# BruceCanovas/supersurfel_fusion

Measured on AMD Instinct MI355X. Metric: frames_per_sec, higher is better.
Workload: dtype f32; 1 GPU; 640x480 synthetic RGB-D orbit (seed 1234), map seeded with 1000000 supersurfels (~993223 live, ~86081 visible), reference rgbd_benchmark parameters, extract+ICP+fuse per frame; width=640, height=480, n_model=993223, n_visible=86081, superpixels=1200, icp_iter_max=10, icp_forced=False, seed_order=seeded, exchange=none, pipeline_depth=2, extract_batch=8

## Files before the change

### supersurfel_fusion_amd/csrc/lab/host_probes.inc

```

int ssf_dbg_last_icp_record(ssf_handle* h, int64_t* out29) {
    if (!h || !out29) return SSF_ERR_INVALID_ARG;
    for (int i = 0; i < 29; i++) out29[i] = h->h_icp_local[i];
    return SSF_OK;
}
int ssf_dbg_device_icp_records(ssf_handle* h, int64_t* out64) {
    if (!h || !out64) return SSF_ERR_INVALID_ARG;
    HCK(hipStreamSynchronize(h->stream));
    HCK(hipMemcpy(out64, h->d_icp, 64 * sizeof(int64_t), hipMemcpyDeviceToHost));
    return SSF_OK;
}
void ssf_dbg_stall_before_match_us(ssf_handle* h, long long us) { if (h) h->dbg_stall_before_match_us = us; }
long long ssf_dbg_assoc_replica_frames(ssf_handle* h) { return h ? h->n_assoc_replica_frames : -1; }
int ssf_dbg_host_times(ssf_handle* h, double* out8) {
    if (!h || !out8) return SSF_ERR_INVALID_ARG;
    for (int i = 0; i < 8; i++) { out8[i] = h->host_us[i]; h->host_us[i] = 0; }
    return SSF_OK;
}
double ssf_dbg_extract_only(ssf_handle* h, const void* const* rgb, const void* const* depth, int nlist, int n) {
    if (!h || !rgb || !depth || nlist <= 0 || !h->pending.empty()) return -1.0;
    int nsub = 0;
    double t0 = 0;
    for (int i = 0; i < n; i++) {
        if (i == n / 4) { for (auto& c : h->ctx) (void)hipStreamSynchronize(c.stream); (void)hipStreamSynchronize(h->stream); t0 = now_us(); }
        while (nsub < n && !h->ctx[h->open_ctx].launched) {
            if (submit_extract(h, rgb[nsub % nlist], depth[nsub % nlist], 1, nullptr)) return -1.0;
            nsub++;
        }
        if (activate_oldest(h) || retire_active(h)) return -1.0;
        h->stamp++;
    }
    for (auto& c : h->ctx) (void)hipStreamSynchronize(c.stream);
    (void)hipStreamSynchronize(h->stream);
    return (now_us() - t0) / (double)(n - n / 4);
}
double ssf_dbg_time_icp(ssf_handle* h, int reps, int dbg) {
// ... 111 lines not shown
```

### supersurfel_fusion_amd/csrc/ssf_handle.hpp

```cpp
#pragma once
#include <algorithm>
#include <cassert>
#include <climits>
#include <cmath>
#include <cstring>
#include <deque>
#include <initializer_list>
#include <map>
#include <string>
#include <utility>
#include <vector>
#include "ssf_device.hpp"
#include "ssf_stage_layout.hpp"
#include "../../include/ssf_render.h"
#include "../../include/ssf_graph.h"
#include "../../include/ssf_graph_solve.h"
#include "../../include/ssf_keyframes.h"
#include "../../include/ssf_motion.h"
#include "../../include/ssf_odometry.h"
#include "../../include/ssf_navgrid.h"
#include "../../include/ssf_track.h"

struct ncclComm; typedef struct ncclComm* ncclComm_t;
struct Uploader;
// ... 241 lines not shown
    BinnedList bl;
    unsigned long long* stats = nullptr; int* cbox = nullptr;
    unsigned char* io = nullptr; size_t io_bytes = 0;
    RayIndex ix{};
    bool built = false; unsigned long long gen = 0; long long recentres = 0; float cell = 0, s = 0; int hash_bits = 0;
    long long rows_indexed = 0, rows_oversize = 0, entries = 0;
};
struct ssf_handle {
    ssf_config cfg;
    int S = 0, gx = 0, gy = 0;
    std::string err;
    hipStream_t stream = nullptr; bool own_stream = false; int stream_prio = 0;
    SegParams seg; Cam cam;
    std::vector<ExtractCtx> ctx; int open_ctx = 0, batch = 1;
    std::deque<std::pair<int, int>> pending;
    ActiveFrame active; ActiveFrame* cc = &active;
    uint32_t extract_ordinal = 0;
    const void* const* seq_rgb = nullptr; const void* const* seq_depth = nullptr; const uint8_t* const* seq_pixmask = nullptr; int seq_next = 0, seq_n = 0, seq_on_device = 0, stamp_bias = 0;
    long long n_waiter_matches = 0;
    int seq_k = 0;
    int seq_batches = 0;
    double us_wait_upload = 0.0;
    Uploader* up = nullptr; bool seq_upload = false;
    int in_color = SSF_COLOR_RGB8, in_depth = SSF_DEPTH_F32_METRES; double in_scale = 1.0;
    ncclComm_t comm = nullptr; int* d_all5 = nullptr;
    int deal = 0; long long deal_batches = 0;
    struct P2P {
        unsigned char* region = nullptr; size_t bytes = 0; bool fine = false;
        bool same_device = false; double timeout_s = 30.0;
        P2PView view{}; bool on = false; std::vector<void*> opened;
        unsigned long long seq_icp = 0, seq_cnt = 0, seq_assoc = 0, seq_migr = 0;
    } p2p;
    unsigned long long all_seq = 0; bool all_pending = false, all_valid = false;
    long long all_cnt[5 * SSF_MAX_RANKS];
    SurfelSoA model[2]; int mcur = 0;
    std::vector<void*> allocs;
    struct Guarded { void* base; size_t bytes, guard; };
    std::vector<Guarded> guarded;
    float* d_bf_in = nullptr; float* d_bf_out = nullptr; float* d_orient9 = nullptr; float* d_frame_orient9 = nullptr;
    long long* d_icp = nullptr;
    uint8_t* d_state = nullptr; int32_t* d_cand = nullptr; Counters* d_cnt = nullptr;
    int32_t* d_migrants = nullptr; PartitionWs fuse_ws{}; bool fuse_first = false, fuse_migrate = false, fusing = false;
    MoveTotals fuse_totals{0, 0, 0, 0}; bool move_totals_on = true;
    OovStore oov[2]; int ocur = 0; int oov_head = 0, oov_tail = 0, oov_live = 0; long long n_recentres = 0;
    uint8_t* d_state_oov = nullptr; uint32_t* d_bc_oov = nullptr;
    uint32_t* d_part = nullptr; uint32_t* d_part_ticket = nullptr; int part_words = 0, part_sup_vis = 0, part_sup_oov = 0, part_set = 0;
// ... 106 lines not shown
```

### supersurfel_fusion_amd/csrc/ssf_host.hip

```cpp
#include <atomic>
#include <chrono>
#include <cstdio>
#include <cstdlib>
#include <new>
#include <condition_variable>
#include <mutex>
#include <thread>
#include <type_traits>
#include <unistd.h>
#include "ssf_exchange.hpp"
#include "ssf_solvers.hpp"

using namespace ssf;

namespace ssf {
static thread_local KernelTimer* g_timer = nullptr;
KernelTimer* current_timer() { return g_timer; }
void set_current_timer(KernelTimer* t) { g_timer = t; }
void timer_begin(KernelTimer* t, const char* name, hipStream_t st) {
    KernelTimer::Rec r;
    if (!t->pool_free.empty()) { r = t->pool_free.back(); t->pool_free.pop_back(); }
    else { (void)hipEventCreate(&r.e0); (void)hipEventCreate(&r.e1); }
    r.name = name;
    (void)hipEventRecord(r.e0, st);
    t->open.push_back(r);
}
void timer_end(KernelTimer* t, hipStream_t st) {
    KernelTimer::Rec r = t->open.back(); t->open.pop_back();
    (void)hipEventRecord(r.e1, st);
    t->pending.push_back(r);
}
static void timer_calibrate(KernelTimer* t, hipStream_t st) {
    if (t->bracket_bias_ms >= 0.0) return;
    hipEvent_t e[2 * 16];
    for (auto& x : e) (void)hipEventCreate(&x);
    for (int i = 0; i < 16; i++) { (void)hipEventRecord(e[2 * i], st); (void)hipEventRecord(e[2 * i + 1], st); }
// ... 317 lines not shown
        NCK(api->GroupStart());
        ncclResult_t bc_rc = ncclSuccess;
        for (int b = 0; b < nb && bc_rc == ncclSuccess; b++) {
            const size_t off = (size_t)b * c.maps.slab;
            int32_t* lab = slab_shift(c.maps.label, off); float* pd = slab_shift(c.maps.plane_depth, off); float* w = slab_shift(c.d_wire, off);
            bc_rc = api->Broadcast(lab, lab, P, ncclInt32, root, c.deal_comm, st);
            if (bc_rc == ncclSuccess) bc_rc = api->Broadcast(pd, pd, P, ncclFloat32, root, c.deal_comm, st);
            if (bc_rc == ncclSuccess) bc_rc = api->Broadcast(w, w, 26 * (size_t)h->S, ncclFloat32, root, c.deal_comm, st);
        }
        const ncclResult_t end_rc = api->GroupEnd();
        if (extract_rc) return extract_rc;
        NCK(bc_rc); NCK(end_rc);
        if (!mine || h->deal == 2) launch_import_frame(st, h->seg, c.maps, nb, c.frame, c.d_wire, c.d_best, c.d_matched);
    }
    HCK(hipGetLastError());
    if (c.timed) HCK(hipEventRecord(c.ev_t1, st));
    if (multi) HCK(hipEventRecord(c.ev_done, st));
    if (multi && h->pass_team) h->team_prev = &c;
    c.launched = true; c.waited = false; c.inflight = nb; c.nb_launched = nb;
    h->open_ctx = (int)((&c - h->ctx.data() + 1) % (ptrdiff_t)h->ctx.size());
    if (h->seq_n > 0) {
        if (h->seq_launches < 32) { h->seq_launch_us[h->seq_launches] = t_launch0 - h->seq_t0_us; h->seq_launch_host_us[h->seq_launches] = now_us() - t_launch0; h->seq_launch_n[h->seq_launches++] = nb; }
        h->seq_batches++;
    }
    return SSF_OK;
}
static size_t color_bpp(const ssf_handle* h) { return (h->in_color == SSF_COLOR_RGBA8 || h->in_color == SSF_COLOR_BGRA8) ? 4 : 3; }
static size_t depth_bpp(const ssf_handle* h) { return h->in_depth == SSF_DEPTH_U16_SCALED ? 2 : 4; }
static bool device_input_aligned(ssf_handle* h, const void* rgb, const void* depth) {
    const size_t ca = color_bpp(h) == 4 ? 4 : 1, da = depth_bpp(h);
    if ((rgb && (uintptr_t)rgb % ca) || (depth && (uintptr_t)depth % da)) {
        h->err = "device frame pointer not aligned for the input format (4-byte colour: 4 bytes; depth: its element size)";
        return false;
    }
    return true;
}
static bool frame_args_ok(ssf_handle* h, const void* rgb, const void* depth, int on_device) {
    return h && rgb && depth && (!on_device || device_input_aligned(h, rgb, depth));
}
static int submit_extract(ssf_handle* h, const void* rgb, const void* depth, int on_device, const uint8_t* mask,
                          const uint8_t* pixmask = nullptr, int pixmask_on_device = 0) {
    ExtractCtx& c = h->ctx[h->open_ctx];
    if (c.launched) { h->err = "extract pipeline is full: process a submitted frame first"; return SSF_ERR_STATE; }
    if (on_device && !device_input_aligned(h, rgb, depth)) return SSF_ERR_INVALID_ARG;
    const int b = c.count;
    if (b == 0) {
        c.stamp0 = h->stamp + h->stamp_bias + (int)h->pending.size(); c.mask_bits = 0; c.pixmask_bits = 0; c.epoch0 = h->extract_ordinal;
        c.from_tables = false;
        if (h->deal && h->comm) { c.deal_batch = h->deal_batches++; c.mine = (int)(c.deal_batch % (long long)h->cfg.nranks) == h->cfg.rank; }
        else c.mine = true;
    }
    h->extract_ordinal++;
    const size_t P = (size_t)h->cfg.width * h->cfg.height, off = (size_t)b * c.maps.slab;
    c.in.rgb[b] = (const uint8_t*)rgb; c.in.depth[b] = depth;
    if (!on_device && c.mine) {
        uint8_t* drgb = slab_shift(c.d_rgb_in, off); float* ddep = slab_shift(c.d_depth_in, off);
        HCK(hipMemcpyAsync(drgb, rgb, color_bpp(h) * P, hipMemcpyHostToDevice, c.stream));
        HCK(hipMemcpyAsync(ddep, depth, depth_bpp(h) * P, hipMemcpyHostToDevice, c.stream));
        c.in.rgb[b] = drgb; c.in.depth[b] = ddep;
    }
    if (mask && c.mine) { HCK(hipMemcpyAsync(slab_shift(c.d_mask, off), mask, h->S, hipMemcpyHostToDevice, c.stream)); c.mask_bits |= 1u << b; }
    if (pixmask && c.mine) {
        HCK(hipMemcpyAsync(slab_shift(c.d_pixmask, off), pixmask, P, pixmask_on_device ? hipMemcpyDeviceToDevice : hipMemcpyHostToDevice, c.stream));
        c.pixmask_bits |= 1u << b;
    }
    c.count = b + 1;
    h->pending.push_back(std::make_pair(h->open_ctx, b));
    if (c.count == (h->seq_n > 0 ? seq_batch_size(h->seq_batches, h->batch) : h->batch)) return launch_batch(h, c);
    return SSF_OK;
}
static int submit_tables(ssf_handle* h, const int32_t* label, const float* plane_depth, const ssf_surfels* fr, int on_device) {
    if (h->ctx[h->open_ctx].count > 0 && !h->ctx[h->open_ctx].launched) {
        int rc = launch_batch(h, h->ctx[h->open_ctx]);
        if (rc) return rc;
    }
    ExtractCtx& c = h->ctx[h->open_ctx];
    if (c.launched) { h->err = "extract pipeline is full: process a submitted frame first"; return SSF_ERR_STATE; }
    hipStream_t st = c.stream;
    const bool multi = h->ctx.size() > 1;
    if (multi && c.consumed_valid) HCK(hipStreamWaitEvent(st, c.ev_consumed, 0));
    c.stamp0 = h->stamp + h->stamp_bias + (int)h->pending.size(); c.mask_bits = 0; c.pixmask_bits = 0; c.epoch0 = h->extract_ordinal;
    h->extract_ordinal++;
    c.from_tables = true;
    const size_t P = (size_t)h->cfg.width * h->cfg.height, S = (size_t)h->S;
    const hipMemcpyKind kind = on_device ? hipMemcpyDeviceToDevice : hipMemcpyHostToDevice;
    c.timed = false;
    HCK(hipMemcpyAsync(c.maps.label, label, 4 * P, kind, st));
    HCK(hipMemcpyAsync(c.maps.plane_depth, plane_depth, 4 * P, kind, st));
    float* w = c.d_wire;
    HCK(hipMemcpyAsync(w, fr->positions, 12 * S, kind, st)); w += 3 * S;
    HCK(hipMemcpyAsync(w, fr->colors, 12 * S, kind, st)); w += 3 * S;
    HCK(hipMemcpyAsync(w, fr->stamps, 8 * S, kind, st)); w += 2 * S;
    HCK(hipMemcpyAsync(w, fr->orientations, 36 * S, kind, st)); w += 9 * S;
    HCK(hipMemcpyAsync(w, fr->shapes, 24 * S, kind, st)); w += 6 * S;
    HCK(hipMemcpyAsync(w, fr->dims, 8 * S, kind, st)); w += 2 * S;
    HCK(hipMemcpyAsync(w, fr->confidences, 4 * S, kind, st));
    if (!on_device) HCK(hipStreamSynchronize(st));
    launch_import_frame(st, h->seg, c.maps, 1, c.frame, c.d_wire, c.d_best, c.d_matched);
    HCK(hipGetLastError());
    if (multi) HCK(hipEventRecord(c.ev_done, st));
    c.count = 1; c.launched = true; c.waited = false; c.inflight = 1; c.nb_launched = 1;
    h->pending.push_back(std::make_pair(h->open_ctx, 0));
    h->open_ctx = (int)((&c - h->ctx.data() + 1) % (ptrdiff_t)h->ctx.size());
    return SSF_OK;
}
static int retire_active(ssf_handle* h) {
    ExtractCtx* c = h->active.ctx;
    if (!c || !h->have_frame) return SSF_OK;
    h->have_frame = false;
    if (--c->inflight == 0) {
        if (h->ctx.size() > 1) { HCK(hipEventRecord(c->ev_consumed, h->stream)); c->consumed_valid = true; }
        c->launched = false; c->count = 0;
    }
    return SSF_OK;
}
static int activate_oldest(ssf_handle* h) {
    if (h->fusing) { h->err = "a frame is between ssf_stage_fuse_begin and ssf_stage_fuse_end"; return SSF_ERR_STATE; }
    if (h->pending.empty()) { h->err = "no submitted frame"; return SSF_ERR_STATE; }
    int rc = retire_active(h);
    if (rc) return rc;
    const std::pair<int, int> fr = h->pending.front();
    ExtractCtx& c = h->ctx[fr.first];
    if (!c.launched) { rc = launch_batch(h, c); if (rc) return rc; }
    h->pending.pop_front();
    if (h->ctx.size() > 1 && !c.waited) { HCK(hipStreamWaitEvent(h->stream, c.ev_done, 0)); c.waited = true; }
    if (c.stamp0 + fr.second != h->stamp) { h->err = "submitted frame is out of sequence (model stamp changed while frames were pending)"; return SSF_ERR_STATE; }
    const size_t off = (size_t)fr.second * c.maps.slab;
    ActiveFrame& a = h->active;
    a.maps = batch_slot(c.maps, fr.second); a.frame = batch_slot(c.frame, off);
    a.d_best = slab_shift(c.d_best, off); a.d_matched = slab_shift(c.d_matched, off);
    a.ctx = &c; a.slot = fr.second; a.pixmask = ((c.pixmask_bits >> fr.second) & 1u) != 0;
    a.has_rgba = !c.from_tables && c.mine; a.activated = true;
    h->have_frame = true;
    return SSF_OK;
}
static int seq_flush_tail(ssf_handle* h) {
    if (h->seq_next < h->seq_n) return SSF_OK;
    ExtractCtx& c = h->ctx[h->open_ctx];
    return (c.count > 0 && !c.launched) ? launch_batch(h, c) : SSF_OK;
}
static int seq_submit(ssf_handle* h) {
    const int i = h->seq_next;
    const uint8_t* pixmask = h->seq_pixmask ? h->seq_pixmask[i] : nullptr;
    if (h->seq_on_device || !h->seq_upload) {
        int rc = submit_extract(h, h->seq_rgb[i], h->seq_depth[i], h->seq_on_device, nullptr, pixmask, h->seq_on_device);
        if (!rc) { h->seq_next++; rc = seq_flush_tail(h); }
        return rc;
    }
    Uploader& u = *h->up;
    const auto t0 = std::chrono::steady_clock::now();
    const double w0 = now_us();
    for (unsigned long long spins = 0; !u.ready(i); spins++) {
        if (u.failed.load()) { h->err = "upload of a host frame failed"; return SSF_ERR_DEVICE; }
        if ((spins & 0xFFFF) == 0xFFFF && std::chrono::duration<double>(std::chrono::steady_clock::now() - t0).count() > 10.0) {
            h->err = "upload of a host frame never finished"; return SSF_ERR_DEVICE;
        }
        std::this_thread::yield();
    }
    h->us_wait_upload += now_us() - w0;
    const int sl = i % u.ring;
    int rc = submit_extract(h, u.d_rgb[sl], u.d_depth[sl], 1, nullptr, pixmask ? u.d_mask[sl] : nullptr, 1);
    if (!rc) { h->seq_next++; rc = seq_flush_tail(h); }
    return rc;
}
static int do_extract(ssf_handle* h, const void* rgb, const void* depth, int on_device, const uint8_t* mask, const uint8_t* pixmask = nullptr) {
    if (!frame_args_ok(h, rgb, depth, on_device)) return SSF_ERR_INVALID_ARG;
    TimerScope ts(h);
    if (!h->pending.empty()) { h->err = "frames are pending in the extract pipeline"; return SSF_ERR_STATE; }
    int rc = retire_active(h);
    if (!rc) rc = submit_extract(h, rgb, depth, on_device, mask, pixmask, on_device);
    return rc ? rc : activate_oldest(h);
}

static inline bool single_shard_alone(const ssf_handle* h) { return h->cfg.nranks == 1 && !h->comm && !h->p2p.on; }
static inline bool exchanges_natively(const ssf_handle* h) { return h->comm || h->p2p.on; }
static inline bool icp_is_one_launch(const ssf_handle* h) { return single_shard_alone(h) || (h->p2p.on && !h->comm); }
static inline long long total_model(const ssf_handle* h) { return (h->cfg.nranks > 1 && h->global_n_model >= 0) ? h->global_n_model : h->n_model; }
static inline long long total_visible(const ssf_handle* h) { return (h->cfg.nranks > 1 && h->global_n_visible >= 0) ? h->global_n_visible : h->n_visible; }
static void icp_start_from(IcpLoop& I, const Rt& pose) {
// ... 249 lines not shown
        launch_fuse(h->stream, M, h->cc->frame, h->pose, h->stamp, h->id_offset, h->n_visible, at, nvis_g > 0 ? 1 : 0,
                    h->cfg.nb_supersurfels_max, h->shard, h->d_cnt, h->oov[h->ocur], h->oov_tail - h->oov_head, h->classify,
                    h->d_state, h->d_state_oov, h->d_bc_oov, ws, h->fuse_totals.from_tot);
        if (h->fuse_migrate)
            launch_pack_emigrants(h->stream, M, at, h->id_offset, h->n_visible, h->d_state, nvis_g > 0 ? 1 : 0, h->shard, h->d_migrants);
    }
    HCK(hipGetLastError());
    h->fusing = true;
    h->model_gen++;
    return SSF_OK;
}
static int fuse_end(ssf_handle* h, const int32_t* d_table, ssf_frame_result* out) {
    SurfelSoA& M = h->model[h->mcur];
    const unsigned long long seq = ++h->cnt_seq;
    h->fusing = false;
    if (!h->fuse_first) {
        const PartitionWs& ws = h->fuse_ws;
        if (h->fuse_migrate && d_table)
            launch_migrate_in(h->stream, M, d_table, h->S, h->cfg.nb_supersurfels_max, h->d_cnt, h->shard, h->classify, h->pose, h->stamp,
                              h->d_state, ws);
        NextIcp next{};
        P2PView next_pv{};
        bool have_next = false;
        if (h->icp_ahead && (h->p2p.on || h->ahead_tuner.current() == 1) && icp_is_one_launch(h) && h->cfg.icp_iter > 0 && !h->pending.empty()) {
            ExtractCtx& nc = h->ctx[h->pending.front().first];
            const int nslot = h->pending.front().second;
            const bool multi = h->ctx.size() > 1;
            bool ready = nc.launched && (!multi || nc.waited);
            if (nc.launched && !ready && (h->icp_ahead_mode == 2 || h->p2p.on || hipEventQuery(nc.ev_done) == hipSuccess)) {
                HCK(hipStreamWaitEvent(h->stream, nc.ev_done, 0)); nc.waited = true; ready = true;
            }
            (void)hipGetLastError();
            if (ready) {
                const FrameMaps nm = batch_slot(nc.maps, nslot);
                IcpLoop first;
                icp_start_from(first, h->pose);
                next = NextIcp{h->cam, nm.pix2, nm.fpack, icp_transform(first), h->d_icp_replicas, h->d_tickets + 8, h->d_icp, h->mb_dev, ++h->icp_seq};
                if (h->p2p.on) next_pv = p2p_view(h, ++h->p2p.seq_icp);
                h->ahead.valid = true; h->ahead.seq = next.seq; h->ahead.ctx = &nc; h->ahead.slot = nslot;
                h->ahead.stamp = h->stamp + 1; h->ahead.pose = h->pose;
                have_next = true;
            }
        }
        if (exchanges_natively(h)) { int rg = comm_gather_counts(h); if (rg) return rg; }
        launch_move_rows(h->stream, M, h->model[h->mcur ^ 1], h->oov[h->ocur], h->n_visible + (h->fuse_migrate ? 2 : 1) * h->S, h->oov_tail - h->oov_head,
                         h->d_state, h->d_state_oov, h->d_bc_oov, ws, h->d_cnt, h->mb_dev, seq, have_next ? &next : nullptr,
                         have_next && h->p2p.on ? &next_pv : nullptr, h->fuse_totals.from_tot ? &h->fuse_totals : nullptr);
        h->mcur ^= 1;
    } else {
        launch_first_frame(h->stream, M, h->cc->frame, h->pose, h->S, h->cfg.nb_supersurfels_max, h->shard, h->d_cnt);
        launch_publish_counts(h->stream, h->d_cnt, 0, h->mb_dev, seq);
        if (exchanges_natively(h)) { int rg = comm_gather_counts(h); if (rg) return rg; }
    }
    HCK(hipGetLastError());
    { int rr = retire_active(h); if (rr) return rr; }
    h->stamp_bias = 1;
    while (h->seq_next < h->seq_n && !h->ctx[h->open_ctx].launched) {
        int rs = seq_submit(h);
        if (rs) { h->stamp_bias = 0; return rs; }
    }
    h->stamp_bias = 0;
    int rc = wait_seq(h, &h->mb_host->cnt_seq, seq);
    if (rc) return rc;
    Counters c;
    for (int attempt = 0;; attempt++) {
        unsigned long long check = seq;
        const int* srcw = reinterpret_cast<const int*>(&h->mb_host->cnt);
        int* dstw = reinterpret_cast<int*>(&c);
        for (int i = 0; i < (int)(sizeof(Counters) / sizeof(int)); i++) {
            dstw[i] = __atomic_load_n(&srcw[i], __ATOMIC_RELAXED);
            check += (unsigned long long)(unsigned int)dstw[i];
        }
        if (check == __atomic_load_n(&h->mb_host->cnt_check, __ATOMIC_ACQUIRE)) break;
        if (attempt > 100000) { h->err = "counter mailbox record failed its checksum"; return SSF_ERR_DEVICE; }
    }
    h->n_model = c.n_model; h->n_visible = c.n_visible;
    h->oov_head = c.oov_head; h->oov_tail = c.oov_tail; h->oov_live = c.oov_live;
    if (__atomic_load_n(&h->mb_host->extract_abort, __ATOMIC_ACQUIRE) != 0u) {
        __atomic_store_n(&h->mb_host->extract_abort, 0u, __ATOMIC_RELEASE);
        h->err = "a team launch of the relabelling passes could not get all its workgroups onto the GPU and gave up (the GPU is oversubscribed: "
                 "several processes?); the frames of that batch are invalid";
        return SSF_ERR_DEVICE;
    }
    if (h->p2p.on && __atomic_load_n(&h->mb_host->p2p_timeout, __ATOMIC_ACQUIRE) != 0u) {
        __atomic_store_n(&h->mb_host->p2p_timeout, 0u, __ATOMIC_RELEASE);
        h->err = "a peer's association / migrant tables never arrived (peer-to-peer exchange)"; return SSF_ERR_DEVICE;
// ... 38 lines not shown
    h->wait_launched_us = now_us();
    Rt none; none.R = m3_identity(); none.t = v3(0, 0, 0);
    const P2PView pv = h->p2p.view;
    const MatchArgs ma{h->cfg.range_min, h->cfg.range_max, h->id_offset, h->cc->d_best, h->cc->d_matched, h->d_cand, h->assoc_rstride};
    const int rc = icp_issue(h, none, w.seq_rec, nullptr, w.slot, w.go_seq, h->p2p.on ? &pv : nullptr, icp_waiter_can_match(h) ? &ma : nullptr);
    w.waiting = rc == SSF_OK;
    return rc;
}
static bool icp_resident_ok(const ssf_handle* h) {
    return h->go_res && single_shard_alone(h) && !h->bins.valid && !h->cfg.depth_prefilter && icp_variant_mode() == 0 && h->n_visible > 0 &&
           h->n_visible <= h->resident_max_rows;
}
static int icp_launch_resident(ssf_handle* h, IcpWaiter& w, const Rt* T0, unsigned long long seq0) {
    const int last = h->cfg.icp_iter;
    IcpGo* lines = h->go_res + (size_t)(h->n_resident_launches++ & 1) * (size_t)(last + 1);
    const unsigned long long go_base = h->go_count;
    h->go_count += (unsigned long long)last;
    w.resident = true; w.slot = lines + 1; w.go_seq = go_base + 1;
    h->wait_launched_us = now_us();
    const MatchArgs ma{h->cfg.range_min, h->cfg.range_max, h->id_offset, h->cc->d_best, h->cc->d_matched, h->d_cand, h->assoc_rstride};
    launch_icp_resident(h->stream, h->cam, h->model[h->mcur], h->n_visible, h->cc->maps.pix2, h->cc->maps.fpack, T0, h->d_icp_replicas, h->d_icp, h->mb_dev,
                        seq0, lines, (unsigned int)go_base, last, icp_waiter_can_match(h) ? &ma : nullptr);
    HCK(hipGetLastError());
    w.waiting = true;
    if (!w.resident_counted) { w.resident_counted = true; h->n_resident_frames++; if (!T0) h->n_resident_ahead_frames++; }
    return SSF_OK;
}
static void icp_resident_iterate(ssf_handle* h, IcpWaiter& w, const Rt& T, unsigned long long seq_rec) {
    h->wait_launched_us = now_us();
    icp_release_waiting(w.slot, w.go_seq, &T, seq_rec);
    w.slot++; w.go_seq++;
}
static void icp_chain_reset(ssf_handle* h) {
    (void)hipStreamSynchronize(h->stream);
    (void)hipMemsetAsync(h->d_icp_replicas, 0, 2 * SSF_ICP_REPLICAS * 32 * sizeof(long long), h->stream);
    (void)hipMemsetAsync(h->d_tickets, 0, 512 * sizeof(unsigned int), h->stream);
    (void)hipStreamSynchronize(h->stream);
    h->icp_chain = false; h->ahead.valid = false;
}
struct TrackFrame { double t_a = 0.0, t_b = 0.0; int kf = -1; bool timing = false, first_it = true; IcpWaiter w; };
int TileCopy::make_if_large(ssf_handle* h) {
    if (!(h->icp.active && min_rows >= 0 && h->n_visible >= min_rows && h->n_visible > 0 && single_shard_alone(h) && bin_buffer_words(h->cam, 1) != 0)) return SSF_OK;
    if (!d_idx) {
        const size_t N = (size_t)h->cfg.nb_supersurfels_max, bw = bin_buffer_words(h->cam, N);
        const bool ok = bw && dalloc(h, &rows.pos, 12 * N) && dalloc(h, &d_idx, 1) && dalloc(h, &d_count, bw) && dalloc(h, &d_cursor, bw);
        if (!ok) { h->err = "allocation of the tile-sorted copy failed"; return SSF_ERR_DEVICE; }
// ... 121 lines not shown
    ExtractCtx* ec = h->cc->ctx;
    if (hipEventElapsedTime(&ms, ec->ev_t0, ec->ev_t1) == hipSuccess) r->stage_ms[0] = ms / (float)ec->nb_launched;
    if (hipEventElapsedTime(&ms, h->ev[1], h->ev[2]) == hipSuccess) r->stage_ms[1] = ms;
    if (hipEventElapsedTime(&ms, h->ev[2], h->ev[3]) == hipSuccess) r->stage_ms[2] = ms;
    return SSF_OK;
}

static int process_oldest(ssf_handle* h, const float* prior, ssf_frame_result* out) {
    TimerScope ts(h);
    int rc = activate_oldest(h);
    if (rc) return rc;
    TrackFrame f;
    f.t_a = now_us();
    f.kf = h->seq_n > 0 ? h->seq_k : -1;
    if (f.kf >= 0 && f.kf < 64) { h->seq_mark_us[0][f.kf] = f.t_a - h->seq_t0_us; h->seq_mark_us[1][f.kf] = 0; }
    if (h->ctx.size() > 1 && hipEventQuery(h->cc->ctx->ev_done) == hipSuccess) h->host_us[4] += 1;
    f.timing = h->cfg.profile != 0 && h->cc->ctx->timed;
    if (f.timing) HCK(hipEventRecord(h->ev[1], h->stream));
    if (exchanges_natively(h)) { rc = comm_counts(h); if (rc) return rc; }
    icp_begin(h, prior);
    rc = h->bins.make_if_large(h);
    h->assoc_rstride = rc ? 0 : assoc_replica_stride(h);
    if (!rc) rc = icp_chains(h) ? icp_loop_chained(h, f) : icp_loop_plain(h, f);
    if (!rc) rc = icp_loop_end(h, f);
    ssf_frame_result r;
    if (!rc) rc = exchange_and_fuse(h, &r);
    h->assoc_rstride = 0;
    if (rc) return rc;
    if (h->pending.empty()) h->ahead_tuner.sequence_break(); else h->ahead_tuner.frame_done(now_us(), r.icp_iters);
    h->host_us[1] += f.t_b - f.t_a; h->host_us[2] += now_us() - f.t_b; h->host_us[3] += 1;
    if (f.timing) { rc = stage_times(h, &r); if (rc) return rc; }
    if (out) *out = r;
    return SSF_OK;
}
static int process_frame_impl(ssf_handle* h, const void* rgb, const void* depth, int on_device, const float* prior,
                              const uint8_t* mask, ssf_frame_result* out, const uint8_t* pixmask = nullptr, int pixmask_on_device = -1) {
    if (!frame_args_ok(h, rgb, depth, on_device)) return SSF_ERR_INVALID_ARG;
    if (!h->pending.empty()) { h->err = "frames are pending in the extract pipeline: use ssf_process_submitted"; return SSF_ERR_STATE; }
    int rc;
    { TimerScope ts(h); rc = submit_extract(h, rgb, depth, on_device, mask, pixmask, pixmask_on_device < 0 ? on_device : pixmask_on_device); }
    return rc ? rc : process_oldest(h, prior, out);
}

namespace ssf {
bool frame_inputs_ok(ssf_handle* h, const void* rgb, const void* depth, int on_device) { return frame_args_ok(h, rgb, depth, on_device); }
int process_frame_devmask(ssf_handle* h, const void* rgb, const void* depth, int on_device, const float* prior, const uint8_t* d_pixmask,
                          ssf_frame_result* out) {
    return process_frame_impl(h, rgb, depth, on_device ? 1 : 0, prior, nullptr, out, d_pixmask, 1);
}
int copy_rows(ssf_handle* h, const ssf_surfels& dst, size_t d0, const ssf_surfels& src, size_t s0, size_t n, hipMemcpyKind kind) {
    if (n == 0) return SSF_OK;
    auto one = [&](auto* d, const auto* s, size_t w) { return d ? hipMemcpyAsync(d + w * d0, s + w * s0, 4 * w * n, kind, h->stream) : hipSuccess; };
// ... 98 lines not shown
}

extern "C" {

int ssf_abi_version(void) { return SSF_ABI_VERSION; }
const char* ssf_backend_name(void) { return "hip-gfx950"; }

void ssf_default_config(ssf_config* c) {
    std::memset(c, 0, sizeof(*c));
    c->width = 640; c->height = 480; c->fx = 525.f; c->fy = 525.f; c->cx = 319.5f; c->cy = 239.5f;
    c->cell_size = 16; c->lambda_pos = 50.f; c->lambda_bound = 1000.f; c->lambda_size = 10000.f;
    c->lambda_disp = 1e6f; c->thresh_disp = 1e-4f; c->seg_iter = 10; c->seg_use_ransac = 1;
    c->nb_samples = 16; c->filter_iter = 4; c->filter_alpha = 0.1f; c->filter_beta = 1.0f;
    c->filter_threshold = 0.05f; c->range_min = 0.2f; c->range_max = 5.0f; c->delta_t = 20;
    c->conf_thresh = 2500.f; c->nb_supersurfels_max = 50000; c->icp_iter = 10; c->icp_cov_thresh = 0.04;
    c->rng_seed = 1234; c->icp_force_iters = 0; c->device_id = 0; c->stream = nullptr;
    c->rank = 0; c->nranks = 1; c->shard_tile = 0.5f; c->profile = 0;
    c->depth_prefilter = 1; c->prefilter_sigma_color = 0.03f; c->prefilter_sigma_space = 4.5f;
    c->pipeline_depth = 0; c->extract_batch = 1;
}

void ssf_destroy(ssf_handle* h) {
    if (!h) return;
    if (h->up) {
        h->up->stop.store(1);
        h->up->join();
        h->up->shutdown();
        for (auto q : h->up->p_rgb) if (q) (void)hipHostFree(q);
        for (auto q : h->up->p_depth) if (q) (void)hipHostFree(q);
        for (auto q : h->up->p_mask) if (q) (void)hipHostFree(q);
        delete h->up; h->up = nullptr;
    }
    for (auto& c : h->ctx) if (c.stream) (void)hipStreamSynchronize(c.stream);
    if (h->stream) (void)hipStreamSynchronize(h->stream);
    for (auto& c : h->ctx) if (c.deal_comm) { RcclApi* api = rccl_api(); if (api) (void)api->CommDestroy(c.deal_comm); c.deal_comm = nullptr; }
    if (h->comm) { RcclApi* api = rccl_api(); if (api) (void)api->CommDestroy(h->comm); h->comm = nullptr; }
    for (void* q : h->p2p.opened) (void)hipIpcCloseMemHandle(q);
    if (h->p2p.region) (void)hipFree(h->p2p.region);
    for (auto& c : h->ctx) {
        for (int n = 0; n <= SSF_MAX_BATCH; n++) { if (c.exec[n]) (void)hipGraphExecDestroy(c.exec[n]); if (c.graph[n]) (void)hipGraphDestroy(c.graph[n]); }
        for (int n = 0; n <= SSF_MAX_BATCH; n++) { if (c.exec_pm[n]) (void)hipGraphExecDestroy(c.exec_pm[n]); if (c.graph_pm[n]) (void)hipGraphDestroy(c.graph_pm[n]); }
        hipEvent_t evs[4] = {c.ev_done, c.ev_consumed, c.ev_t0, c.ev_t1};
        for (hipEvent_t e : evs) if (e) (void)hipEventDestroy(e);
        if (c.own_stream && c.stream) stream_pool().give(c.stream, h->cfg.device_id, c.stream_prio);
    }
    if (h->capture_stream) stream_pool().give(h->capture_stream, h->cfg.device_id, StreamPool::CAPTURE);
// ... 190 lines not shown
int ssf_process_frame(ssf_handle* h, const uint8_t* rgb, const float* depth, const float* prior, const uint8_t* mask, ssf_frame_result* out) { return process_frame_impl(h, rgb, depth, 0, prior, mask, out); }
int ssf_process_frame_device(ssf_handle* h, const void* rgb, const void* depth, const float* prior, const uint8_t* mask, ssf_frame_result* out) { return process_frame_impl(h, rgb, depth, 1, prior, mask, out); }

static int submit_frame(ssf_handle* h, const void* rgb, const void* depth, int on_device, const uint8_t* mask, const uint8_t* pixmask) {
    if (!frame_args_ok(h, rgb, depth, on_device)) return SSF_ERR_INVALID_ARG;
    TimerScope ts(h);
    const double t0 = now_us();
    int rc = submit_extract(h, rgb, depth, on_device, mask, pixmask, on_device);
    h->host_us[0] += now_us() - t0;
    return rc;
}
int ssf_submit_frame(ssf_handle* h, const void* rgb, const void* depth, int on_device, const uint8_t* mask) { return submit_frame(h, rgb, depth, on_device, mask, nullptr); }
int ssf_submit_frame_tables(ssf_handle* h, const int32_t* label, const float* plane_depth, const ssf_surfels* frame, int on_device) {
    if (!h || !label || !plane_depth || !frame) return SSF_ERR_INVALID_ARG;
    if (!frame->positions || !frame->colors || !frame->stamps || !frame->orientations || !frame->shapes || !frame->dims || !frame->confidences) return SSF_ERR_INVALID_ARG;
    if (h->deal != 0) { h->err = "ssf_submit_frame_tables: the handle deals its extract stage (ssf_comm_deal_extract); submit frames, not tables"; return SSF_ERR_STATE; }
    TimerScope ts(h);
    return submit_tables(h, label, plane_depth, frame, on_device);
}
int ssf_process_submitted(ssf_handle* h, const float* prior, ssf_frame_result* out) {
    if (!h) return SSF_ERR_INVALID_ARG;
    return process_oldest(h, prior, out);
}
static int process_sequence_impl(ssf_handle* h, const void* const* rgb, const void* const* depth, const uint8_t* const* pixmasks, int n,
                                 int on_device, ssf_frame_result* out) {
    if (!h || !rgb || !depth || n < 0) return SSF_ERR_INVALID_ARG;
    if (!h->pending.empty()) { h->err = "frames are pending in the extract pipeline"; return SSF_ERR_STATE; }
    for (int i = 0; i < n; i++) if (!rgb[i] || !depth[i]) return SSF_ERR_INVALID_ARG;
    if (on_device) for (int i = 0; i < n; i++) if (!device_input_aligned(h, rgb[i], depth[i])) return SSF_ERR_INVALID_ARG;
    int rc = SSF_OK;
    if (h->ctx.size() > 1 && !h->ctx[h->open_ctx].launched && h->ctx[h->open_ctx].count == 0) {
        bool idle = true;
        for (auto& c : h->ctx) idle = idle && !c.launched && c.count == 0;
        if (idle) h->open_ctx = 0;
    }
    const bool ahead = !on_device && h->ctx.size() > 1 && n > 1;
    if (ahead) {
        const size_t P = (size_t)h->cfg.width * h->cfg.height;
        if (!h->up) {
            Uploader* u = new (std::nothrow) Uploader();
            if (!u) { h->err = "out of memory"; return SSF_ERR_DEVICE; }
            const int window = ((int)h->ctx.size() + 1) * h->batch + 2;
            const int by_bytes = (int)(SSF_UPLOAD_RING_BYTES / (8 * P));
            u->ring = std::max(window, std::min(((int)h->ctx.size() + 3) * h->batch + 2, by_bytes));
            u->device = h->cfg.device_id;
            bool ok = true;
// ... 8 lines not shown
                          hipHostMalloc((void**)&u->p_mask[i], P, hipHostMallocDefault) == hipSuccess;
                if (!pin) {
                    for (auto q : u->p_rgb) if (q) (void)hipHostFree(q);
                    for (auto q : u->p_depth) if (q) (void)hipHostFree(q);
                    for (auto q : u->p_mask) if (q) (void)hipHostFree(q);
                    u->p_rgb.clear(); u->p_depth.clear(); u->p_mask.clear(); (void)hipGetLastError();
                }
            }
            for (auto& c : h->ctx) u->ctx_stream.push_back(c.stream);
            u->batch = h->batch;
            if (!ok) { delete u; h->err = "allocation of the upload ring failed"; return SSF_ERR_DEVICE; }
            h->up = u;
        }
        Uploader& u = *h->up;
        u.n = n; u.rgb = rgb; u.depth = depth; u.ctx0 = h->open_ctx;
        u.rgb_bytes = color_bpp(h) * P; u.depth_bytes = depth_bpp(h) * P;
        u.masks = pixmasks; u.mask_bytes = P;
        u.processed.store(0); u.failed.store(0); u.stop.store(0);
        u.start();
    }
    h->seq_rgb = rgb; h->seq_depth = depth; h->seq_pixmask = pixmasks; h->seq_next = 0; h->seq_n = n; h->seq_on_device = on_device; h->seq_upload = ahead;
    h->seq_batches = 0; h->seq_launches = 0;
    h->seq_t0_us = now_us();
    for (int k = 0; k < n && !rc; k++) {
        while (!rc && h->seq_next < n && !h->ctx[h->open_ctx].launched) {
            TimerScope ts(h);
            rc = seq_submit(h);
        }
        h->seq_k = k;
        if (!rc) rc = process_oldest(h, nullptr, out ? &out[k] : nullptr);
        if (k < 64) h->seq_done_us[k] = h->seq_mark_us[3][k] = now_us() - h->seq_t0_us;
        if (ahead) h->up->processed.store(k + 1, std::memory_order_release);
    }
    if (ahead) {
        h->up->stop.store(1);
        h->up->join();
    }
    h->seq_rgb = nullptr; h->seq_depth = nullptr; h->seq_pixmask = nullptr; h->seq_n = 0; h->seq_next = 0; h->seq_upload = false;
    if (h->up) h->up->masks = nullptr;
    return rc;
}
int ssf_process_sequence(ssf_handle* h, const void* const* rgb, const void* const* depth, int n, int on_device, ssf_frame_result* out) {
    return process_sequence_impl(h, rgb, depth, nullptr, n, on_device, out);
}
int ssf_pending_frames(const ssf_handle* h) { return h ? (int)h->pending.size() : 0; }
int ssf_pipeline_capacity(const ssf_handle* h) { return h ? (int)h->ctx.size() * h->batch : 0; }
int ssf_can_submit(const ssf_handle* h) { return (h && !h->ctx[h->open_ctx].launched) ? 1 : 0; }

int ssf_align(ssf_handle* h, const ssf_surfels* src, int n, const float* init_pose, float* rel_pose, int* valid, int* iters,
              int* pairs_last) {
    if (!h || !src || n < 0 || !rel_pose || !valid || !src->positions || !src->colors || !src->orientations) return SSF_ERR_INVALID_ARG;
    TimerScope ts(h);
    const size_t N = (size_t)std::max(n, 1);
    std::vector<float> lab(3 * N), nrm(3 * N);
    for (int i = 0; i < n; i++) {
        const V3 l = rgb_to_lab(v3(src->colors[3 * i], src->colors[3 * i + 1], src->colors[3 * i + 2]));
        lab[3 * i] = l.x; lab[3 * i + 1] = l.y; lab[3 * i + 2] = l.z;
        for (int c = 0; c < 3; c++) nrm[3 * i + c] = src->orientations[9 * i + 6 + c];
    }
    float *d_pos = nullptr, *d_lab = nullptr, *d_nrm = nullptr, *d_conf = nullptr; long long* d_out = nullptr;
// ... 487 lines not shown
```

Measured before the change: 12380 frames/s.

## Move extract batch submission to a dedicated launcher thread during sequences

Adds a background batch-launcher thread with a mutex/condvar queue that submits and launches extract batches while the main thread runs ICP and fusion. The main thread polls or waits for published batches and hands retired contexts back, so extract launch cost on the host comes off the per-frame critical path. In exchange it adds cross-thread synchronisation, spin-then-block waits, thread-local error slots, and more complex stamp/epoch bookkeeping that could race or add latency.

```diff
diff --git a/supersurfel_fusion_amd/csrc/lab/host_probes.inc b/supersurfel_fusion_amd/csrc/lab/host_probes.inc
--- a/supersurfel_fusion_amd/csrc/lab/host_probes.inc
+++ b/supersurfel_fusion_amd/csrc/lab/host_probes.inc
@@ -12,6 +12,31 @@
 }
 void ssf_dbg_stall_before_match_us(ssf_handle* h, long long us) { if (h) h->dbg_stall_before_match_us = us; }
 long long ssf_dbg_assoc_replica_frames(ssf_handle* h) { return h ? h->n_assoc_replica_frames : -1; }
+int ssf_dbg_batch_launcher(ssf_handle* h, double* out16) {
+    if (!h || !out16) return SSF_ERR_INVALID_ARG;
+    for (int i = 0; i < 16; i++) out16[i] = 0.0;
+    if (BatchLauncher* L = launcher_of(h)) {
+        long long np = 0, nw = 0; double us = 0.0;
+        L->q.counters(&np, &nw, &us);
+        if (h->seq_probe.threaded) { out16[0] = (double)np; out16[1] = (double)nw; out16[2] = us; }
+    }
+    const ssf_handle::SeqProbe& sp = h->seq_probe;
+    const double free_us = sp.cnt_n[0] ? sp.cnt_us[0] / (double)sp.cnt_n[0] : 0.0;
+    double sum = 0.0, over = 0.0;
+    for (float v : sp.launch_us) { sum += v; over += std::max(0.0, (double)v - free_us); }
+    out16[3] = (double)sp.launch_us.size();
+    if (!sp.launch_us.empty()) { out16[4] = sum / (double)sp.launch_us.size(); out16[5] = over / (double)sp.launch_us.size(); }
+    for (int c = 0; c < 2; c++) {
+        out16[6 + c] = (double)sp.cnt_n[c]; out16[8 + c] = sp.cnt_n[c] ? sp.cnt_us[c] / (double)sp.cnt_n[c] : 0.0;
+        out16[10 + c] = (double)sp.period_n[c]; out16[12 + c] = sp.period_n[c] ? sp.period_us[c] / (double)sp.period_n[c] : 0.0;
+    }
+    return SSF_OK;
+}
+int ssf_dbg_batch_thread(ssf_handle* h, int on) {
+    if (!h || h->seq_n > 0) return SSF_ERR_INVALID_ARG;
+    h->batch_thread = on != 0;
+    return SSF_OK;
+}
 int ssf_dbg_host_times(ssf_handle* h, double* out8) {
     if (!h || !out8) return SSF_ERR_INVALID_ARG;
     for (int i = 0; i < 8; i++) { out8[i] = h->host_us[i]; h->host_us[i] = 0; }
diff --git a/supersurfel_fusion_amd/csrc/ssf_batch_queue.hpp b/supersurfel_fusion_amd/csrc/ssf_batch_queue.hpp
--- /dev/null
+++ b/supersurfel_fusion_amd/csrc/ssf_batch_queue.hpp
@@ -0,0 +1,119 @@
+#pragma once
+#include <atomic>
+#include <chrono>
+#include <condition_variable>
+#include <deque>
+#include <mutex>
+#include <string>
+
+namespace {
+struct BatchMsg { int ctx, count, first; };
+
+class BatchQueue {
+public:
+    static const int MAX_CTX = 32;
+    enum Take { GOT = 0, FAILED = 1, ENDED = 2 };
+
+    void open(const bool* busy0, int nctx) {
+        {
+            std::lock_guard<std::mutex> lk(mu);
+            ready.clear(); n_ready.store(0, std::memory_order_relaxed);
+            for (int c = 0; c < MAX_CTX; c++) busy[c] = c < nctx ? busy0[c] : true;
+            stopping = false; stop_flag.store(false, std::memory_order_relaxed);
+            rc = 0; err.clear();
+            published = 0; waits = 0; wait_us = 0.0;
+            running = true; gen++;
+        }
+        cv.notify_all();
+    }
+    bool poll(BatchMsg* m) {
+        if (n_ready.load(std::memory_order_acquire) == 0) return false;
+        std::lock_guard<std::mutex> lk(mu);
+        return pop(m);
+    }
+    Take take(BatchMsg* m) {
+        {
+            std::lock_guard<std::mutex> lk(mu);
+            if (pop(m)) return GOT;
+            if (rc) return FAILED;
+            if (!running) return ENDED;
+            waits++;
+        }
+        const auto t0 = std::chrono::steady_clock::now();
+        for (int spins = 0; n_ready.load(std::memory_order_acquire) == 0 && !stop_flag.load(std::memory_order_acquire); spins++) {
+            if ((spins & 63) == 63 && std::chrono::duration<double, std::micro>(std::chrono::steady_clock::now() - t0).count() > SPIN_US) break;
+        }
+        std::unique_lock<std::mutex> lk(mu);
+        cv.wait(lk, [&] { return !ready.empty() || rc != 0 || !running; });
+        wait_us += std::chrono::duration<double, std::micro>(std::chrono::steady_clock::now() - t0).count();
+        if (pop(m)) return GOT;
+        return rc ? FAILED : ENDED;
+    }
+    void retire(int c) {
+        { std::lock_guard<std::mutex> lk(mu); busy[c] = false; }
+        cv.notify_all();
+    }
+    void stop() {
+        { std::lock_guard<std::mutex> lk(mu); stopping = true; stop_flag.store(true, std::memory_order_release); }
+        cv.notify_all();
+    }
+    void wait_idle() { std::unique_lock<std::mutex> lk(mu); cv.wait(lk, [&] { return !running; }); }
+    int error(std::string* text) { std::lock_guard<std::mutex> lk(mu); if (rc && text) *text = err; return rc; }
+    void shutdown() {
+        { std::lock_guard<std::mutex> lk(mu); quit = true; stopping = true; stop_flag.store(true, std::memory_order_release); }
+        cv.notify_all();
+    }
+    void counters(long long* n_published, long long* n_waits, double* us) {
+        std::lock_guard<std::mutex> lk(mu);
+        *n_published = published; *n_waits = waits; *us = wait_us;
+    }
+
+    bool next_job() {
+        std::unique_lock<std::mutex> lk(mu);
+        cv.wait(lk, [&] { return quit || gen != seen; });
+        if (quit) return false;
+        seen = gen;
+        return true;
+    }
+    bool acquire(int c) {
+        std::unique_lock<std::mutex> lk(mu);
+        cv.wait(lk, [&] { return stopping || !busy[c]; });
+        return !stopping;
+    }
+    void publish(const BatchMsg& m) {
+        {
+            std::lock_guard<std::mutex> lk(mu);
+            busy[m.ctx] = true; ready.push_back(m); published++;
+            n_ready.store((int)ready.size(), std::memory_order_release);
+        }
+        cv.notify_all();
+    }
+    void fail(int code, const std::string& text) {
+        { std::lock_guard<std::mutex> lk(mu); rc = code; err = text; stopping = true; stop_flag.store(true, std::memory_order_release); }
+        cv.notify_all();
+    }
+    void done() {
+        { std::lock_guard<std::mutex> lk(mu); running = false; stop_flag.store(true, std::memory_order_release); }
+        cv.notify_all();
+    }
+    bool stop_requested() const { return stop_flag.load(std::memory_order_acquire); }
+
+private:
+    static constexpr double SPIN_US = 200.0;
+    bool pop(BatchMsg* m) {
+        if (ready.empty()) return false;
+        *m = ready.front(); ready.pop_front();
+        n_ready.store((int)ready.size(), std::memory_order_release);
+        return true;
+    }
+    std::mutex mu; std::condition_variable cv;
+    std::deque<BatchMsg> ready;
+    bool busy[MAX_CTX] = {};
+    bool stopping = false, running = false, quit = false;
+    int rc = 0; std::string err;
+    unsigned long long gen = 0, seen = 0;
+    long long published = 0, waits = 0; double wait_us = 0.0;
+    std::atomic<int> n_ready{0};
+    std::atomic<bool> stop_flag{false};
+};
+}
diff --git a/supersurfel_fusion_amd/csrc/ssf_handle.hpp b/supersurfel_fusion_amd/csrc/ssf_handle.hpp
--- a/supersurfel_fusion_amd/csrc/ssf_handle.hpp
+++ b/supersurfel_fusion_amd/csrc/ssf_handle.hpp
@@ -287,6 +287,16 @@
     int seq_batches = 0;
     double us_wait_upload = 0.0;
     Uploader* up = nullptr; bool seq_upload = false;
+    void* launcher = nullptr; bool seq_threaded = false; int seq_retired = -1;
+    bool batch_thread = true;
+    int seq_stamp0 = 0; uint32_t seq_epoch0 = 0;
+#ifdef SSF_EXPERIMENTS
+    struct SeqProbe {
+        std::vector<float> launch_us;
+        double cnt_us[2] = {0, 0}, period_us[2] = {0, 0}, last_done_us = -1.0; long long cnt_n[2] = {0, 0}, period_n[2] = {0, 0};
+        bool freed = false, threaded = false;
+    } seq_probe;
+#endif
     int in_color = SSF_COLOR_RGB8, in_depth = SSF_DEPTH_F32_METRES; double in_scale = 1.0;
     ncclComm_t comm = nullptr; int* d_all5 = nullptr;
     int deal = 0; long long deal_batches = 0;
diff --git a/supersurfel_fusion_amd/csrc/ssf_host.hip b/supersurfel_fusion_amd/csrc/ssf_host.hip
--- a/supersurfel_fusion_amd/csrc/ssf_host.hip
+++ b/supersurfel_fusion_amd/csrc/ssf_host.hip
@@ -10,8 +10,21 @@
 #include <unistd.h>
 #include "ssf_exchange.hpp"
 #include "ssf_solvers.hpp"
+#include "ssf_batch_queue.hpp"
 
 using namespace ssf;
+
+static thread_local std::string* tl_err = nullptr;
+static inline std::string& err_slot(ssf_handle* h) { return tl_err ? *tl_err : h->err; }
+#undef HCK
+#define HCK(call)                                                                                    \
+    do {                                                                                             \
+        hipError_t e_ = (call);                                                                      \
+        if (e_ != hipSuccess) {                                                                      \
+            err_slot(h) = std::string(#call) + ": " + hipGetErrorString(e_);                         \
+            return SSF_ERR_DEVICE;                                                                   \
+        }                                                                                            \
+    } while (0)
 
 namespace ssf {
 static thread_local KernelTimer* g_timer = nullptr;
@@ -375,6 +388,9 @@
     if (h->seq_n > 0) {
         if (h->seq_launches < 32) { h->seq_launch_us[h->seq_launches] = t_launch0 - h->seq_t0_us; h->seq_launch_host_us[h->seq_launches] = now_us() - t_launch0; h->seq_launch_n[h->seq_launches++] = nb; }
         h->seq_batches++;
+#ifdef SSF_EXPERIMENTS
+        h->seq_probe.launch_us.push_back((float)(now_us() - t_launch0));
+#endif
     }
     return SSF_OK;
 }
@@ -394,11 +410,13 @@
 static int submit_extract(ssf_handle* h, const void* rgb, const void* depth, int on_device, const uint8_t* mask,
                           const uint8_t* pixmask = nullptr, int pixmask_on_device = 0) {
     ExtractCtx& c = h->ctx[h->open_ctx];
-    if (c.launched) { h->err = "extract pipeline is full: process a submitted frame first"; return SSF_ERR_STATE; }
-    if (on_device && !device_input_aligned(h, rgb, depth)) return SSF_ERR_INVALID_ARG;
+    if (c.launched) { err_slot(h) = "extract pipeline is full: process a submitted frame first"; return SSF_ERR_STATE; }
+    if (on_device && !h->seq_threaded && !device_input_aligned(h, rgb, depth)) return SSF_ERR_INVALID_ARG;
     const int b = c.count;
     if (b == 0) {
-        c.stamp0 = h->stamp + h->stamp_bias + (int)h->pending.size(); c.mask_bits = 0; c.pixmask_bits = 0; c.epoch0 = h->extract_ordinal;
+        if (h->seq_threaded) { c.stamp0 = h->seq_stamp0 + h->seq_next; c.epoch0 = h->seq_epoch0 + (uint32_t)h->seq_next; }
+        else { c.stamp0 = h->stamp + h->stamp_bias + (int)h->pending.size(); c.epoch0 = h->extract_ordinal; }
+        c.mask_bits = 0; c.pixmask_bits = 0;
         c.from_tables = false;
         if (h->deal && h->comm) { c.deal_batch = h->deal_batches++; c.mine = (int)(c.deal_batch % (long long)h->cfg.nranks) == h->cfg.rank; }
         else c.mine = true;
@@ -418,7 +436,7 @@
         c.pixmask_bits |= 1u << b;
     }
     c.count = b + 1;
-    h->pending.push_back(std::make_pair(h->open_ctx, b));
+    if (!h->seq_threaded) h->pending.push_back(std::make_pair(h->open_ctx, b));
     if (c.count == (h->seq_n > 0 ? seq_batch_size(h->seq_batches, h->batch) : h->batch)) return launch_batch(h, c);
     return SSF_OK;
 }
@@ -457,6 +475,54 @@
     h->open_ctx = (int)((&c - h->ctx.data() + 1) % (ptrdiff_t)h->ctx.size());
     return SSF_OK;
 }
+namespace {
+struct BatchLauncher {
+    BatchQueue q;
+    std::thread th;
+    std::string err;
+    int device = 0;
+};
+}
+static inline BatchLauncher* launcher_of(const ssf_handle* h) { return static_cast<BatchLauncher*>(h->launcher); }
+static inline void seq_hand_over_retired(ssf_handle* h) {
+    if (h->seq_retired >= 0) { launcher_of(h)->q.retire(h->seq_retired); h->seq_retired = -1; }
+}
+static const int SEQ_STOPPED = 1 << 20;
+static int seq_submit(ssf_handle* h);
+static void launcher_main(ssf_handle* h, BatchLauncher* L) {
+    tl_err = &L->err;
+    const bool dev_ok = hipSetDevice(L->device) == hipSuccess;
+    while (L->q.next_job()) {
+        int rc = SSF_OK;
+        if (!dev_ok) { rc = SSF_ERR_DEVICE; L->err = "hipSetDevice failed on the batch launcher's thread"; }
+        bool stopped = false;
+        while (!rc && !stopped && h->seq_next < h->seq_n) {
+            const int c0 = h->open_ctx, first = h->seq_next;
+            if (!L->q.acquire(c0)) break;
+            ExtractCtx& c = h->ctx[c0];
+            while (!rc && !c.launched && h->seq_next < h->seq_n) rc = seq_submit(h);
+            if (rc == SEQ_STOPPED) { stopped = true; rc = (c.count > 0 && !c.launched) ? launch_batch(h, c) : SSF_OK; }
+            if (!rc && c.launched) L->q.publish(BatchMsg{c0, c.count, first});
+        }
+        if (rc) L->q.fail(rc, L->err);
+        L->q.done();
+    }
+}
+static void seq_list_batch(ssf_handle* h, const BatchMsg& m) {
+    for (int b = 0; b < m.count; b++) h->pending.push_back(std::make_pair(m.ctx, b));
+}
+static void seq_poll_batches(ssf_handle* h) {
+    BatchMsg m;
+    while (launcher_of(h)->q.poll(&m)) seq_list_batch(h, m);
+}
+static int seq_wait_batch(ssf_handle* h) {
+    seq_hand_over_retired(h);
+    BatchMsg m;
+    const BatchQueue::Take t = launcher_of(h)->q.take(&m);
+    if (t == BatchQueue::GOT) { seq_list_batch(h, m); return SSF_OK; }
+    if (t == BatchQueue::FAILED) return launcher_of(h)->q.error(&h->err);
+    h->err = "no submitted frame"; return SSF_ERR_STATE;
+}
 static int retire_active(ssf_handle* h) {
     ExtractCtx* c = h->active.ctx;
     if (!c || !h->have_frame) return SSF_OK;
@@ -464,11 +530,16 @@
     if (--c->inflight == 0) {
         if (h->ctx.size() > 1) { HCK(hipEventRecord(c->ev_consumed, h->stream)); c->consumed_valid = true; }
         c->launched = false; c->count = 0;
+        if (h->seq_threaded) { seq_hand_over_retired(h); h->seq_retired = (int)(c - h->ctx.data()); }
+#ifdef SSF_EXPERIMENTS
+        h->seq_probe.freed = true;
+#endif
     }
     return SSF_OK;
 }
 static int activate_oldest(ssf_handle* h) {
     if (h->fusing) { h->err = "a frame is between ssf_stage_fuse_begin and ssf_stage_fuse_end"; return SSF_ERR_STATE; }
+    if (h->pending.empty() && h->seq_threaded) { const int rw = seq_wait_batch(h); if (rw) return rw; }
     if (h->pending.empty()) { h->err = "no submitted frame"; return SSF_ERR_STATE; }
     int rc = retire_active(h);
     if (rc) return rc;
@@ -504,10 +575,11 @@
     const auto t0 = std::chrono::steady_clock::now();
     const double w0 = now_us();
     for (unsigned long long spins = 0; !u.ready(i); spins++) {
-        if (u.failed.load()) { h->err = "upload of a host frame failed"; return SSF_ERR_DEVICE; }
+        if (u.failed.load()) { err_slot(h) = "upload of a host frame failed"; return SSF_ERR_DEVICE; }
         if ((spins & 0xFFFF) == 0xFFFF && std::chrono::duration<double>(std::chrono::steady_clock::now() - t0).count() > 10.0) {
-            h->err = "upload of a host frame never finished"; return SSF_ERR_DEVICE;
-        }
+            err_slot(h) = "upload of a host frame never finished"; return SSF_ERR_DEVICE;
+        }
+        if (h->seq_threaded && launcher_of(h)->q.stop_requested()) return SEQ_STOPPED;
         std::this_thread::yield();
     }
     h->us_wait_upload += now_us() - w0;
@@ -803,6 +875,7 @@
         NextIcp next{};
         P2PView next_pv{};
         bool have_next = false;
+        if (h->seq_threaded) seq_poll_batches(h);
         if (h->icp_ahead && (h->p2p.on || h->ahead_tuner.current() == 1) && icp_is_one_launch(h) && h->cfg.icp_iter > 0 && !h->pending.empty()) {
             ExtractCtx& nc = h->ctx[h->pending.front().first];
             const int nslot = h->pending.front().second;
@@ -834,15 +907,24 @@
         if (exchanges_natively(h)) { int rg = comm_gather_counts(h); if (rg) return rg; }
     }
     HCK(hipGetLastError());
+#ifdef SSF_EXPERIMENTS
+    const double t_moved = now_us();
+    h->seq_probe.freed = false;
+#endif
     { int rr = retire_active(h); if (rr) return rr; }
-    h->stamp_bias = 1;
-    while (h->seq_next < h->seq_n && !h->ctx[h->open_ctx].launched) {
-        int rs = seq_submit(h);
-        if (rs) { h->stamp_bias = 0; return rs; }
-    }
-    h->stamp_bias = 0;
+    if (!h->seq_threaded) {
+        h->stamp_bias = 1;
+        while (h->seq_next < h->seq_n && !h->ctx[h->open_ctx].launched) {
+            int rs = seq_submit(h);
+            if (rs) { h->stamp_bias = 0; return rs; }
+        }
+        h->stamp_bias = 0;
+    }
     int rc = wait_seq(h, &h->mb_host->cnt_seq, seq);
     if (rc) return rc;
+#ifdef SSF_EXPERIMENTS
+    if (h->seq_n > 0) { const int cls = h->seq_probe.freed ? 1 : 0; h->seq_probe.cnt_us[cls] += now_us() - t_moved; h->seq_probe.cnt_n[cls]++; }
+#endif
     Counters c;
     for (int attempt = 0;; attempt++) {
         unsigned long long check = seq;
@@ -927,6 +1009,7 @@
     launch_icp_resident(h->stream, h->cam, h->model[h->mcur], h->n_visible, h->cc->maps.pix2, h->cc->maps.fpack, T0, h->d_icp_replicas, h->d_icp, h->mb_dev,
                         seq0, lines, (unsigned int)go_base, last, icp_waiter_can_match(h) ? &ma : nullptr);
     HCK(hipGetLastError());
+    if (h->seq_threaded) seq_hand_over_retired(h);
     w.waiting = true;
     if (!w.resident_counted) { w.resident_counted = true; h->n_resident_frames++; if (!T0) h->n_resident_ahead_frames++; }
     return SSF_OK;
@@ -1094,12 +1177,14 @@
     rc = h->bins.make_if_large(h);
     h->assoc_rstride = rc ? 0 : assoc_replica_stride(h);
     if (!rc) rc = icp_chains(h) ? icp_loop_chained(h, f) : icp_loop_plain(h, f);
+    if (h->seq_threaded) seq_hand_over_retired(h);
     if (!rc) rc = icp_loop_end(h, f);
     ssf_frame_result r;
     if (!rc) rc = exchange_and_fuse(h, &r);
     h->assoc_rstride = 0;
     if (rc) return rc;
-    if (h->pending.empty()) h->ahead_tuner.sequence_break(); else h->ahead_tuner.frame_done(now_us(), r.icp_iters);
+    const bool more = !h->pending.empty() || (h->seq_threaded && h->seq_k + 1 < h->seq_n);
+    if (!more) h->ahead_tuner.sequence_break(); else h->ahead_tuner.frame_done(now_us(), r.icp_iters);
     h->host_us[1] += f.t_b - f.t_a; h->host_us[2] += now_us() - f.t_b; h->host_us[3] += 1;
     if (f.timing) { rc = stage_times(h, &r); if (rc) return rc; }
     if (out) *out = r;
@@ -1244,6 +1329,11 @@
 
 void ssf_destroy(ssf_handle* h) {
     if (!h) return;
+    if (BatchLauncher* L = launcher_of(h)) {
+        L->q.shutdown();
+        if (L->th.joinable()) L->th.join();
+        delete L; h->launcher = nullptr;
+    }
     if (h->up) {
         h->up->stop.store(1);
         h->up->join();
@@ -1480,6 +1570,44 @@
     if (!h) return SSF_ERR_INVALID_ARG;
     return process_oldest(h, prior, out);
 }
+static int launcher_start(ssf_handle* h) {
+    BatchLauncher* L = launcher_of(h);
+    if (!L) {
+        L = new (std::nothrow) BatchLauncher();
+        if (!L) { h->err = "out of memory"; return SSF_ERR_DEVICE; }
+        L->device = h->cfg.device_id;
+        L->th = std::thread(launcher_main, h, L);
+        h->launcher = L;
+    }
+    bool busy[BatchQueue::MAX_CTX] = {};
+    for (size_t c = 0; c < h->ctx.size(); c++) busy[c] = h->ctx[c].launched;
+    h->seq_stamp0 = h->stamp; h->seq_epoch0 = h->extract_ordinal;
+    L->err.clear();
+    h->seq_threaded = true;
+#ifdef SSF_EXPERIMENTS
+    h->seq_probe.threaded = true;
+#endif
+    L->q.open(busy, (int)h->ctx.size());
+    return SSF_OK;
+}
+static int launcher_finish(ssf_handle* h, int rc) {
+    BatchLauncher* L = launcher_of(h);
+    if (rc) L->q.stop();
+    seq_hand_over_retired(h);
+    L->q.wait_idle();
+    h->seq_threaded = false;
+    BatchMsg m;
+    while (L->q.poll(&m)) seq_list_batch(h, m);
+    ExtractCtx& oc = h->ctx[h->open_ctx];
+    if (oc.count > 0 && !oc.launched) for (int b = 0; b < oc.count; b++) h->pending.push_back(std::make_pair(h->open_ctx, b));
+    if (!rc) rc = L->q.error(&h->err);
+    return rc;
+}
+static void launcher_abandon_uploads(ssf_handle* h, bool ahead) {
+    if (!ahead) return;
+    h->up->stop.store(1);
+    h->up->join();
+}
 static int process_sequence_impl(ssf_handle* h, const void* const* rgb, const void* const* depth, const uint8_t* const* pixmasks, int n,
                                  int on_device, ssf_frame_result* out) {
     if (!h || !rgb || !depth || n < 0) return SSF_ERR_INVALID_ARG;
@@ -1534,20 +1662,34 @@
     h->seq_rgb = rgb; h->seq_depth = depth; h->seq_pixmask = pixmasks; h->seq_next = 0; h->seq_n = n; h->seq_on_device = on_device; h->seq_upload = ahead;
     h->seq_batches = 0; h->seq_launches = 0;
     h->seq_t0_us = now_us();
+#ifdef SSF_EXPERIMENTS
+    h->seq_probe = ssf_handle::SeqProbe();
+#endif
+    static const bool batch_thread = !SSF_ENV_SET("NO_BATCH_THREAD");
+    if (batch_thread && h->batch_thread && n > 0 && h->ctx.size() > 1 && (int)h->ctx.size() <= BatchQueue::MAX_CTX && single_shard_alone(h) && !h->deal &&
+        h->cfg.profile != 1 && h->ctx[h->open_ctx].count == 0) {
+        rc = launcher_start(h);
+    }
     for (int k = 0; k < n && !rc; k++) {
-        while (!rc && h->seq_next < n && !h->ctx[h->open_ctx].launched) {
+        while (!rc && !h->seq_threaded && h->seq_next < n && !h->ctx[h->open_ctx].launched) {
             TimerScope ts(h);
             rc = seq_submit(h);
         }
         h->seq_k = k;
         if (!rc) rc = process_oldest(h, nullptr, out ? &out[k] : nullptr);
         if (k < 64) h->seq_done_us[k] = h->seq_mark_us[3][k] = now_us() - h->seq_t0_us;
+#ifdef SSF_EXPERIMENTS
+        {
+            ssf_handle::SeqProbe& sp = h->seq_probe;
+            const double t_done = now_us();
+            if (sp.last_done_us >= 0.0 && !rc) { sp.period_us[sp.freed ? 1 : 0] += t_done - sp.last_done_us; sp.period_n[sp.freed ? 1 : 0]++; }
+            sp.last_done_us = t_done;
+        }
+#endif
         if (ahead) h->up->processed.store(k + 1, std::memory_order_release);
     }
-    if (ahead) {
-        h->up->stop.store(1);
-        h->up->join();
-    }
+    if (h->seq_threaded) rc = launcher_finish(h, rc);
+    launcher_abandon_uploads(h, ahead);
     h->seq_rgb = nullptr; h->seq_depth = nullptr; h->seq_pixmask = nullptr; h->seq_n = 0; h->seq_next = 0; h->seq_upload = false;
     if (h->up) h->up->masks = nullptr;
     return rc;
```

New measurement: 12380 frames/s. No clear change (-0.0%).
